# Chatit-cloud/BEE2BEE

Hardware: NVIDIA H100
Metric: decode_tokens_per_sec (higher is better)
Workload: dtype bf16

## Files before the change

bee2bee_b200/ops/__init__.py:

```python
from __future__ import annotations

import importlib
import importlib.util
from typing import Optional

import torch

EPI_PLAIN, EPI_RESIDUAL, EPI_GLU, EPI_QKV_ROPE, EPI_GELU = 0, 1, 2, 3, 4
PAGE = 64
NUM_SMS = 132

_C = None

LAUNCHES = [0]
_KERNEL_ENTRY_POINTS = ("add", "attention", "decode_advance", "embed", "fetch_window", "flag_signal", "flag_wait", "gemm",
                        "kv_append", "layernorm", "mark_seen", "quant_fp8_rows", "quant_mxfp8_rows", "rmsnorm", "sample",
                        "set_decode_state")


class _CountedModule:

    def __init__(self, mod):
        self._mod = mod
        for name in dir(mod):
# ... 287 lines not shown


def attention(q, k_cache, v_cache, out, block_table, q_start, q_len, kv_len, *, max_q, n_q, n_kv, head_dim,
              window=0, softcap=0.0, splits=1, ws=None, use_tc=-1, fq_out=None, fq_sf=None, fq_bn=0):
    native().attention(q, k_cache, v_cache, out, block_table, q_start, q_len, kv_len, ws, max_q, n_q, n_kv, head_dim,
                       window, softcap, splits, use_tc, _ptr(fq_out), _ptr(fq_sf), fq_bn)
    if splits > 1:
        LAUNCHES[0] += 1
    return out


def attention_fuses_quant(max_q: int, n_q: int, n_kv: int, head_dim: int, splits: int) -> bool:
    return native().attention_uses_tc(max_q, n_q, n_kv, head_dim) and (max_q > 1 or splits <= 1)


def set_attn_tc_min_q(n: int) -> None:
    native().set_attn_tc_min_q(int(n))


def get_attn_tc_min_q() -> int:
    return int(native().get_attn_tc_min_q())


def sample(logits, out_tokens, *, seen=None, temperature=None, top_p=None, rep_penalty=None, seeds=None, step=None,
           peer_tokens=0, history=0, hist_pos=None, hist_stride=0, signal_flag=0, signal_epoch=0, done_counter=0,
           vocab=0, softcap=0.0, row_map=0):
    native().sample(logits, seen, out_tokens, peer_tokens, history, hist_pos, hist_stride, vocab, softcap,
                    temperature, top_p,
                    rep_penalty, seeds, step, signal_flag, signal_epoch, done_counter, row_map)
    return out_tokens
# ... 5 lines not shown
```

csrc/attention_tc.cu:

```cuda
#include "kernels.h"

#include <cuda.h>
#include <cuda_fp8.h>

#include <cstdlib>
#include <type_traits>

#include "common.cuh"
#include "launch.cuh"
#include "wgmma.cuh"

namespace b2b {

int make_tmap_shared(CUtensorMap* m, const void* ptr, uint64_t rows, uint64_t cols, uint64_t ld, uint32_t box_rows,
                     int elt_bytes);

namespace {

constexpr int APAGE = 64;
constexpr int ATC_CONSUMERS = 256;
constexpr int ATC_THREADS = ATC_CONSUMERS + 32;
constexpr float LOG2E = 1.4426950408889634f;

struct AttnTcParams {
  __nv_bfloat16* out;
  const int* block_table;
  const int* q_start;
  const int* q_len;
  const int* kv_len;
  int max_pages, n_q, n_kv, window;
  float softcap;
  int splits, ws_rows;
  float* ws;
  uint8_t* q_out8;
  uint8_t* q_sf;
  int q_bn;
};

template <int D>
struct AtcCfg {
  static constexpr int BKV = 64;
  static constexpr int kQBytes = 128 * D * 2;
  static constexpr int kKVBytes = BKV * D * 2;
  static constexpr int kSmemBytes = kQBytes + 4 * kKVBytes + 256;
};

template <int D, bool SOFTCAP>
__global__ void __launch_bounds__(ATC_THREADS, 1)
attn_prefill_tc_kernel(const __grid_constant__ CUtensorMap tm_q, const __grid_constant__ CUtensorMap tm_k,
                       const __grid_constant__ CUtensorMap tm_v, const AttnTcParams p, const int G, const int QB) {
  using Cfg = AtcCfg<D>;
  constexpr int BKV = Cfg::BKV;
  constexpr int DB = D / 64;

  extern __shared__ __align__(1024) uint8_t smem[];
  if ((smem_u32(smem) & 1023u) != 0u) __trap();
  uint8_t* q_s = smem;
  uint8_t* k_s = q_s + Cfg::kQBytes;
  uint8_t* v_s = k_s + 2 * Cfg::kKVBytes;
  uint64_t* bars = reinterpret_cast<uint64_t*>(v_s + 2 * Cfg::kKVBytes);
  uint64_t* q_full = bars + 0;
  uint64_t* k_full = bars + 1;
  uint64_t* v_full = bars + 3;
  uint64_t* k_empty = bars + 5;
  uint64_t* v_empty = bars + 7;

  const int warp = threadIdx.x >> 5, lane = threadIdx.x & 31;
// ... 15 lines not shown
  const int qblk = split_mode ? 0 : gridDim.x - 1 - blockIdx.x;
  const int qlen = p.q_len[seq], kvlen = p.kv_len[seq];
  const int q0 = qblk * QB;
  bool active = q0 < qlen;
  const int nq_here = min(QB, qlen - q0);
  const int qtok0 = p.q_start[seq] + q0;
  const int pos0 = kvlen - qlen + q0;
  const int kv_hi = min(kvlen, pos0 + nq_here);
  const int kv_lo = p.window > 0 ? max(0, pos0 - p.window + 1) : 0;
  int t_lo = kv_lo / BKV, t_hi = (kv_hi + BKV - 1) / BKV;
  if (active && split_mode) {
    const int per = (t_hi - t_lo + p.splits - 1) / p.splits;
    t_lo = min(t_hi, t_lo + static_cast<int>(blockIdx.x) * per);
    t_hi = min(t_hi, t_lo + per);
    if (t_hi <= t_lo) {
      if (threadIdx.x < G) {
        float* w = p.ws + (((static_cast<size_t>(seq) * p.n_kv + kvh) * p.splits + blockIdx.x) * p.ws_rows + threadIdx.x) * (D + 2);
        for (int c = 0; c < D; ++c) w[c] = 0.f;
        w[D] = -INFINITY;
        w[D + 1] = 0.f;
      }
      active = false;
    }
  }
  const int nt = t_hi - t_lo;
  if (!active) return;

  if (warp == ATC_CONSUMERS / 32) {
    if (lane == 0) {
      mbar_arrive_expect_tx(q_full, Cfg::kQBytes);
      for (int g = 0; g < G; ++g)
        for (int c = 0; c < DB; ++c)
          tma_load_2d(q_s + c * (128 * 128) + g * QB * 128, &tm_q, q_full, (kvh * G + g) * D + c * 64, qtok0);
      const int* bt = p.block_table + static_cast<size_t>(seq) * p.max_pages;
      for (int n = 0; n < nt; ++n) {
        const int s = n & 1;
// ... 4 lines not shown
#pragma unroll
        for (int c = 0; c < DB; ++c)
          tma_load_2d(k_s + s * Cfg::kKVBytes + c * (BKV * 128), &tm_k, &k_full[s], kvh * D + c * 64, page * APAGE);
        mbar_wait(&v_empty[s], ph ^ 1u);
        mbar_arrive_expect_tx(&v_full[s], Cfg::kKVBytes);
#pragma unroll
        for (int c = 0; c < DB; ++c)
          tma_load_2d(v_s + s * Cfg::kKVBytes + c * (BKV * 128), &tm_v, &v_full[s], kvh * D + c * 64, page * APAGE);
      }
    }
    return;
  }

  const int wg = warp >> 2;
  const int ra = wg * 64 + (warp & 3) * 16 + (lane >> 2);
  int gq[2], iq[2], qpos[2];
  bool valid[2];
#pragma unroll
  for (int h = 0; h < 2; ++h) {
    const int row = ra + 8 * h;
    gq[h] = row / QB;
    iq[h] = row % QB;
    valid[h] = (gq[h] < G) && (iq[h] < nq_here);
    qpos[h] = pos0 + iq[h];
  }
  const float cap = p.softcap;
  const float inv_cap = SOFTCAP ? 1.f / cap : 0.f;
  float m_ref[2] = {-INFINITY, -INFINITY}, l[2] = {0.f, 0.f};
  float o[D / 2];
#pragma unroll
  for (int e = 0; e < D / 2; ++e) o[e] = 0.f;
  auto release = [&](uint64_t* bar) {
    __syncwarp();
    if (lane == 0) mbar_arrive(bar);
  };

  mbar_wait(q_full, 0);
  auto tile = [&](int n, auto masked) {
    const int t = t_lo + n, s = n & 1;
    const uint32_t ph = static_cast<uint32_t>((n >> 1) & 1);
    float sc[BKV / 2];
#pragma unroll
    for (int e = 0; e < BKV / 2; ++e) sc[e] = 0.f;
    mbar_wait(&k_full[s], ph);
    wgmma_fence();
#pragma unroll
    for (int kk = 0; kk < D / 16; ++kk) {
      const uint64_t a = make_sw128_kmajor_desc(smem_u32(q_s + (kk / 4) * (128 * 128) + wg * 64 * 128)) +
                         static_cast<uint64_t>((kk % 4) * 2);
      const uint64_t b = make_sw128_kmajor_desc(smem_u32(k_s + s * Cfg::kKVBytes + (kk / 4) * (BKV * 128))) +
                         static_cast<uint64_t>((kk % 4) * 2);
      Wgmma<BKV>::bf16_ss(sc, a, b, kk > 0 ? 1u : 0u);
    }
    wgmma_commit();
    wgmma_wait<0>();
    wgmma_fence_regs(sc);
    release(&k_empty[s]);

    float mrow[2] = {-INFINITY, -INFINITY};
#pragma unroll
    for (int e = 0; e < BKV / 2; ++e) {
      const int h = (e >> 1) & 1;
      float v = sc[e];
      if constexpr (SOFTCAP) v = cap * tanhf(v * inv_cap);
      v *= LOG2E;
      if constexpr (decltype(masked)::value) {
        const int kvpos = t * BKV + (e >> 2) * 8 + 2 * (lane & 3) + (e & 1);
        const bool ok = valid[h] && kvpos <= qpos[h] && kvpos < kvlen && (p.window <= 0 || kvpos > qpos[h] - p.window);
        v = ok ? v : -INFINITY;
      }
      sc[e] = v;
      mrow[h] = fmaxf(mrow[h], v);
    }
    float alpha[2], mr[2];
#pragma unroll
    for (int h = 0; h < 2; ++h) {
      mrow[h] = fmaxf(mrow[h], __shfl_xor_sync(0xffffffffu, mrow[h], 1));
      mrow[h] = fmaxf(mrow[h], __shfl_xor_sync(0xffffffffu, mrow[h], 2));
      alpha[h] = 1.f;
      if (mrow[h] > m_ref[h] + 8.f || (m_ref[h] == -INFINITY && mrow[h] > -INFINITY)) {
        alpha[h] = (m_ref[h] == -INFINITY) ? 0.f : exp2f(m_ref[h] - mrow[h]);
        m_ref[h] = mrow[h];
      }
      mr[h] = (m_ref[h] == -INFINITY) ? 0.f : m_ref[h];
    }
#pragma unroll
    for (int e = 0; e < D / 2; ++e) o[e] *= alpha[(e >> 1) & 1];
    uint32_t pa[BKV / 16][4];
    float lsum[2] = {0.f, 0.f};
#pragma unroll
    for (int e = 0; e < BKV / 2; e += 2) {
      const int h = (e >> 1) & 1;
      const float p0 = exp2f(sc[e] - mr[h]), p1 = exp2f(sc[e + 1] - mr[h]);
      lsum[h] += p0 + p1;
      const __nv_bfloat162 hv = __floats2bfloat162_rn(p0, p1);
      pa[e / 8][(e % 8) / 2] = *reinterpret_cast<const uint32_t*>(&hv);
    }
    l[0] = l[0] * alpha[0] + lsum[0];
    l[1] = l[1] * alpha[1] + lsum[1];
    mbar_wait(&v_full[s], ph);
    wgmma_fence_regs(o);
    wgmma_fence();
#pragma unroll
    for (int kk = 0; kk < BKV / 16; ++kk) {
      const uint64_t b = make_sw128_mnmajor_desc(smem_u32(v_s + s * Cfg::kKVBytes + kk * (16 * 128)), BKV * 128);
      Wgmma<D>::bf16_rs_tb(o, pa[kk], b, 1u);
    }
    wgmma_commit();
    wgmma_wait<0>();
    wgmma_fence_regs(o);
    release(&v_empty[s]);
  };

  for (int n = 0; n < nt; ++n) {
    const int t = t_lo + n;
    const bool full = nq_here == QB && (t + 1) * BKV - 1 <= pos0 && (t + 1) * BKV <= kvlen &&
                      (p.window <= 0 || t * BKV > pos0 + nq_here - 1 - p.window);
    if (full) tile(n, std::false_type{}); else tile(n, std::true_type{});
  }

#pragma unroll
  for (int h = 0; h < 2; ++h) {
    l[h] += __shfl_xor_sync(0xffffffffu, l[h], 1);
    l[h] += __shfl_xor_sync(0xffffffffu, l[h], 2);
  }
  const int c2 = 2 * (lane & 3);
#pragma unroll
  for (int h = 0; h < 2; ++h) {
    const float inv = l[h] > 0.f ? 1.f / l[h] : 0.f;
    const int tok = qtok0 + iq[h], head = kvh * G + gq[h];
    if (split_mode) {
      if (valid[h]) {
        float* wsrow = p.ws + (((static_cast<size_t>(seq) * p.n_kv + kvh) * p.splits + blockIdx.x) * p.ws_rows + gq[h]) * (D + 2);
        if ((lane & 3) == 0) {
          wsrow[D] = (m_ref[h] == -INFINITY) ? -INFINITY : m_ref[h] * 0.6931471805599453f;
          wsrow[D + 1] = l[h];
        }
#pragma unroll
        for (int j = 0; j < D / 8; ++j)
          *reinterpret_cast<float2*>(wsrow + 8 * j + c2) = make_float2(o[4 * j + 2 * h], o[4 * j + 2 * h + 1]);
      }
    } else if (p.q_out8 != nullptr) {
      const int ldq = p.n_q * D;
#pragma unroll
      for (int b = 0; b < D / 32; ++b) {
        float v[8];
        float amax = 0.f;
#pragma unroll
        for (int jj = 0; jj < 4; ++jj) {
          v[2 * jj] = bf16_round(o[4 * (4 * b + jj) + 2 * h] * inv);
          v[2 * jj + 1] = bf16_round(o[4 * (4 * b + jj) + 2 * h + 1] * inv);
          amax = fmaxf(amax, fmaxf(fabsf(v[2 * jj]), fabsf(v[2 * jj + 1])));
        }
        amax = fmaxf(amax, __shfl_xor_sync(0xffffffffu, amax, 1));
        amax = fmaxf(amax, __shfl_xor_sync(0xffffffffu, amax, 2));
        const uint32_t u = __float_as_uint(amax * (1.f / 448.f));
        int ex = static_cast<int>(u >> 23) - 127 + ((u & 0x7FFFFFu) ? 1 : 0);
        ex = max(-126, min(127, ex));
        const float scl = __uint_as_float(static_cast<uint32_t>(127 - ex) << 23);
        if (valid[h]) {
          const int feat = head * D + 32 * b;
          uint8_t* q8 = p.q_out8 + static_cast<size_t>(tok) * ldq + feat;
#pragma unroll
          for (int jj = 0; jj < 4; ++jj) {
            const uint16_t lo = __nv_cvt_float_to_fp8(v[2 * jj] * scl, __NV_SATFINITE, __NV_E4M3);
            const uint16_t hi = __nv_cvt_float_to_fp8(v[2 * jj + 1] * scl, __NV_SATFINITE, __NV_E4M3);
            *reinterpret_cast<uint16_t*>(q8 + 8 * jj + c2) = static_cast<uint16_t>(lo | (hi << 8));
          }
          if ((lane & 3) == 0) {
            const int tile_i = tok / p.q_bn, n = tok - tile_i * p.q_bn, rr = n & 127;
            p.q_sf[(static_cast<size_t>(tile_i) * (ldq >> 7) + (feat >> 7)) * (p.q_bn > 128 ? 1024 : 512) + (n >> 7) * 512 +
                   (rr & 31) * 16 + (rr >> 5) * 4 + ((feat >> 5) & 3)] = static_cast<uint8_t>(ex + 127);
          }
        }
      }
    } else if (valid[h]) {
      __nv_bfloat16* dst = p.out + (static_cast<size_t>(tok) * p.n_q + head) * D;
#pragma unroll
      for (int j = 0; j < D / 8; ++j)
        *reinterpret_cast<__nv_bfloat162*>(dst + 8 * j + c2) =
            __floats2bfloat162_rn(o[4 * j + 2 * h] * inv, o[4 * j + 2 * h + 1] * inv);
    }
  }
}

template <int D, bool SOFTCAP>
int launch_tc_cap(const CUtensorMap& tq, const CUtensorMap& tk, const CUtensorMap& tv, const AttnTcParams& p, int G, int QB,
                  int seqs, int qblocks, cudaStream_t s) {
  using Cfg = AtcCfg<D>;
  static bool set[64] = {};
  int dev = 0;
  cudaGetDevice(&dev);
  if (dev < 64 && !set[dev]) {
    cudaError_t e = cudaFuncSetAttribute(attn_prefill_tc_kernel<D, SOFTCAP>, cudaFuncAttributeMaxDynamicSharedMemorySize,
                                         Cfg::kSmemBytes);
    if (e != cudaSuccess) return static_cast<int>(e);
    set[dev] = true;
  }
  return static_cast<int>(launch_kernel(attn_prefill_tc_kernel<D, SOFTCAP>,
                                        dim3(p.splits > 1 ? p.splits : qblocks, p.n_kv, seqs), dim3(ATC_THREADS),
                                        Cfg::kSmemBytes, s, 1, tq, tk, tv, p, G, QB));
}

template <int D>
int launch_tc(const CUtensorMap& tq, const CUtensorMap& tk, const CUtensorMap& tv, const AttnTcParams& p, int G, int QB,
              int seqs, int qblocks, cudaStream_t s) {
  return p.softcap > 0.f ? launch_tc_cap<D, true>(tq, tk, tv, p, G, QB, seqs, qblocks, s)
                         : launch_tc_cap<D, false>(tq, tk, tv, p, G, QB, seqs, qblocks, s);
}

}

bool attention_tc_supported(int n_q, int n_kv, int head_dim) {
  if (n_kv <= 0 || n_q % n_kv) return false;
  const int G = n_q / n_kv;
  if (G != 1 && G != 2 && G != 4 && G != 8 && G != 16) return false;
  return head_dim == 64 || head_dim == 128 || head_dim == 256;
}

int launch_attention_tc(const void* q, const void* k_cache, const void* v_cache, void* out, const int* block_table,
                        const int* q_start, const int* q_len, const int* kv_len, int seqs, int max_q, int max_pages,
                        int n_tokens, int n_pages, int n_q, int n_kv, int head_dim, int window, float softcap,
                        int splits, float* ws, void* q_out8, void* q_sf, int q_bn, cudaStream_t s) {
  if (!attention_tc_supported(n_q, n_kv, head_dim)) return -2;
  const int G = n_q / n_kv, QB = 128 / G;
  CUtensorMap tq, tk, tv;
  int r = make_tmap_shared(&tq, q, static_cast<uint64_t>(n_tokens), static_cast<uint64_t>(n_q) * head_dim,
                           static_cast<uint64_t>(n_q) * head_dim, static_cast<uint32_t>(QB), 2);
  if (r) return r;
  const uint64_t kv_rows = static_cast<uint64_t>(n_pages) * APAGE, kv_cols = static_cast<uint64_t>(n_kv) * head_dim;
  if ((r = make_tmap_shared(&tk, k_cache, kv_rows, kv_cols, kv_cols, APAGE, 2))) return r;
  if ((r = make_tmap_shared(&tv, v_cache, kv_rows, kv_cols, kv_cols, APAGE, 2))) return r;
  AttnTcParams p;
  p.out = static_cast<__nv_bfloat16*>(out);
  p.block_table = block_table; p.q_start = q_start; p.q_len = q_len; p.kv_len = kv_len;
  p.max_pages = max_pages; p.n_q = n_q; p.n_kv = n_kv; p.window = window; p.softcap = softcap;
  p.splits = (max_q == 1 && splits > 1 && ws != nullptr) ? splits : 1;
  p.ws = ws;
  p.ws_rows = attn_rows(G, 1);
  p.q_out8 = p.splits > 1 ? nullptr : static_cast<uint8_t*>(q_out8);
  p.q_sf = static_cast<uint8_t*>(q_sf);
  p.q_bn = q_bn > 0 ? q_bn : 32;
  if (q_out8 != nullptr && p.splits > 1) return -8;
  const int qblocks = (max_q + QB - 1) / QB;
  int rc;
  switch (head_dim) {
    case 64: rc = launch_tc<64>(tq, tk, tv, p, G, QB, seqs, qblocks, s); break;
    case 128: rc = launch_tc<128>(tq, tk, tv, p, G, QB, seqs, qblocks, s); break;
    case 256: rc = launch_tc<256>(tq, tk, tv, p, G, QB, seqs, qblocks, s); break;
    default: return -3;
  }
  if (rc == 0 && p.splits > 1)
    rc = launch_attention_merge(out, q_start, q_len, ws, seqs, n_q, n_kv, head_dim, p.splits, s);
  return rc;
}

}
```

csrc/binding.cpp:

```cpp
#include <ATen/cuda/CUDAContext.h>
#include <c10/cuda/CUDAGuard.h>
#include <torch/extension.h>

#include "gemm_tc.cuh"
#include "kernels.h"
#include "launch.cuh"
#include "peer.h"

using at::Tensor;
using OptT = c10::optional<Tensor>;

namespace {

inline cudaStream_t cur_stream() { return at::cuda::getCurrentCUDAStream().stream(); }

inline void check(int err, const char* what) {
  if (err != 0) {
    const char* msg = err > 0 ? cudaGetErrorString(static_cast<cudaError_t>(err)) : "invalid argument";
    TORCH_CHECK(false, what, " failed: code ", err, " (", msg, ")");
  }
}
template <typename T>
inline T* ptr_or_null(const OptT& t) {
  return (t.has_value() && t->defined()) ? reinterpret_cast<T*>(t->data_ptr()) : nullptr;
// ... 270 lines not shown
          "attention_tc");
    return;
  }
  TORCH_CHECK(fq_out == 0, "fused output quantisation needs the tensor-core attention kernel");
  check(b2b::launch_attention(q.data_ptr(), k_cache.data_ptr(), v_cache.data_ptr(), out.data_ptr(),
                              reinterpret_cast<const int*>(block_table.data_ptr()),
                              reinterpret_cast<const int*>(q_start.data_ptr()),
                              reinterpret_cast<const int*>(q_len.data_ptr()),
                              reinterpret_cast<const int*>(kv_len.data_ptr()), ptr_or_null<float>(ws), seqs,
                              static_cast<int>(max_q), static_cast<int>(block_table.size(1)), static_cast<int>(n_q),
                              static_cast<int>(n_kv), static_cast<int>(head_dim), static_cast<int>(window),
                              static_cast<float>(softcap), static_cast<int>(splits), cur_stream()),
        "attention");
}

void sample(const Tensor& logits, const OptT& seen, const Tensor& out_tokens, int64_t peer_tokens,
            int64_t history, const OptT& hist_pos, int64_t hist_stride, int64_t vocab, double softcap,
            const OptT& temperature, const OptT& top_p,
            const OptT& rep_penalty, const OptT& seeds, const OptT& step, int64_t signal_flag, int64_t signal_epoch,
            int64_t done_counter, int64_t row_map) {
  TORCH_CHECK(logits.is_cuda() && logits.scalar_type() == at::kFloat && logits.stride(1) == 1, "logits: fp32");
  c10::cuda::CUDAGuard guard(logits.device());
  int* hp = ptr_or_null<int>(hist_pos);
  check(b2b::launch_sample(reinterpret_cast<const float*>(logits.data_ptr()), ptr_or_null<uint32_t>(seen),
                           reinterpret_cast<int*>(out_tokens.data_ptr()), as_ptr<int>(peer_tokens),
                           as_ptr<int>(history), hp, hp, static_cast<int>(hist_stride),
                           static_cast<int>(logits.size(0)), static_cast<int>(vocab > 0 ? vocab : logits.size(1)),
                           static_cast<int>(logits.stride(0)), static_cast<float>(softcap),
                           ptr_or_null<const float>(temperature), ptr_or_null<const float>(top_p),
                           ptr_or_null<const float>(rep_penalty), ptr_or_null<const uint32_t>(seeds),
// ... 95 lines not shown
  m.def("rmsnorm", &rmsnorm);
  m.def("layernorm", &layernorm);
  m.def("embed", &embed);
  m.def("kv_append", &kv_append);
  m.def("add", &add);
  m.def("quant_fp8_rows", &quant_fp8_rows);
  m.def("quant_mxfp8_rows", &quant_mxfp8_rows);
  m.def("flag_wait", &flag_wait);
  m.def("flag_signal", &flag_signal);
  m.def("decode_advance", &decode_advance);
  m.def("attention", &attention);
  m.def("attention_uses_tc", &attention_uses_tc, py::arg("max_q"), py::arg("n_q"), py::arg("n_kv"), py::arg("head_dim"),
        py::arg("use_tc") = -1);
  m.def("set_attn_tc_min_q", &set_attn_tc_min_q);
  m.def("get_attn_tc_min_q", &get_attn_tc_min_q);
  m.def("sample", &sample);
  m.def("sample_cluster_size", &sample_cluster_size, py::arg("batch"), py::arg("vocab"));
  m.def("mark_seen", &mark_seen);
  m.def("set_decode_state", &set_decode_state);
  m.def("fetch_window", &fetch_window);
  m.def("set_wait_policy", &set_wait_policy);
  m.def("peer_alloc", &peer_alloc);
  m.def("peer_free", &peer_free);
  m.def("ipc_export", &ipc_export);
  m.def("ipc_import", &ipc_import);
  m.def("ipc_close", &ipc_close);
  m.def("enable_peer_access", &enable_peer_access);
  m.def("can_access_peer", &can_access_peer);
  m.def("memcpy_peer", &memcpy_peer);
  m.def("host_ring_alloc", &host_ring_alloc);
// ... 4 lines not shown
```

csrc/gemm_tc.cu:

```cuda
#include "gemm_tc.cuh"

#include <cuda_fp8.h>

#include <cstdio>
#include <map>
#include <mutex>
#include <tuple>

#include "common.cuh"
#include "launch.cuh"
#include "wgmma.cuh"

namespace b2b {

constexpr int BM = 128;
constexpr int BK = 64;
constexpr int ROW_BYTES = 128;
constexpr int A_STAGE_BYTES = BM * ROW_BYTES;
constexpr int GEMM_CONSUMERS = 256;
constexpr int GEMM_THREADS = GEMM_CONSUMERS + 32;

template <int BN>
struct GemmCfg {
  static constexpr int kStages = (BN <= 32) ? 5 : (BN == 64 ? 4 : (BN == 128 ? 6 : 4));
// ... 630 lines not shown
  if ((r = set_attr_epi<BN, EPI_PLAIN>()) || (r = set_attr_epi<BN, EPI_RESIDUAL>()) || (r = set_attr_epi<BN, EPI_GLU>()) ||
      (r = set_attr_epi<BN, EPI_QKV_ROPE>()) || (r = set_attr_epi<BN, EPI_GELU>()))
    return r;
  return 0;
}
int gemm_tc_init() {
  int r = 0;
  if ((r = set_attr_bn<16>())) return r;
  if ((r = set_attr_bn<32>())) return r;
  if ((r = set_attr_bn<64>())) return r;
  if ((r = set_attr_bn<128>())) return r;
  if ((r = set_attr_bn<256>())) return r;
  return get_encode() ? 0 : -1;
}

int gemm_tc_default_stages(int bn) {
  switch (bn) {
    case 16: return GemmCfg<16>::kStages;
    case 32: return GemmCfg<32>::kStages;
    case 64: return GemmCfg<64>::kStages;
    case 128: return GemmCfg<128>::kStages;
    default: return GemmCfg<256>::kStages;
  }
}

int gemm_tc_max_splitk(int bn, int epi, int stages) {
  int ring;
  const int dflt = gemm_tc_default_stages(bn);
  if (stages <= 0 || stages > dflt) stages = dflt;
  if (stages < 2) stages = 2;
// ... 69 lines not shown
```

csrc/kernels.h:

```cpp
#pragma once
#include <cuda_runtime.h>
#include <stddef.h>
#include <stdint.h>

namespace b2b {

int launch_rmsnorm(const void* x, const void* gamma, const void* residual, void* out, float* rstd_out, int tokens,
                   int h, float eps, int gemma_plus_one, cudaStream_t s);
int launch_layernorm(const void* x, const void* gamma, const void* beta, void* out, int tokens, int h, float eps,
                     cudaStream_t s);
int launch_embed(const int* ids, const void* table, const void* pos_table, const int* positions, void* out, int tokens,
                 int h, int vocab, float scale, const uint32_t* tok_flag, const uint32_t* tok_epoch, const uint32_t* pf_flag,
                 const uint32_t* pf_need, cudaStream_t s);
int launch_kv_append(const void* qkv, void* q_out, void* k_cache, void* v_cache, const int* slots, int tokens,
                     int q_dim, int kv_dim, float q_scale, cudaStream_t s);
int launch_add(const void* a, const void* b, void* out, size_t n, cudaStream_t s);
int launch_quant_fp8_rows(const void* x, void* q, float* scale_out, int tokens, int h, float eps, int with_rms,
                          cudaStream_t s);
int launch_quant_mxfp8_rows(const void* x, void* q, void* sf, int tokens, int h, int bn, float eps, int with_rms,
                            float* sumsq_out, cudaStream_t s);
int launch_flag_wait(const uint32_t* flag, const uint32_t* epoch, uint32_t delta, cudaStream_t s);
int launch_decode_advance(int* positions, int* kv_len, int* slots, const int* q_len, const int* block_table,
                          int max_pages, int n, cudaStream_t s);
int launch_flag_signal(uint32_t* flag, uint32_t* epoch, uint32_t* bump_epoch, uint32_t* ack_flag, cudaStream_t s);

int launch_attention(const void* q, const void* k_cache, const void* v_cache, void* out, const int* block_table,
                     const int* q_start, const int* q_len, const int* kv_len, float* ws, int seqs, int max_q,
                     int max_pages, int n_q, int n_kv, int head_dim, int window, float softcap, int splits,
                     cudaStream_t s);
int attn_rows(int G, int QB);
bool attention_tc_supported(int n_q, int n_kv, int head_dim);
int launch_attention_tc(const void* q, const void* k_cache, const void* v_cache, void* out, const int* block_table,
                        const int* q_start, const int* q_len, const int* kv_len, int seqs, int max_q, int max_pages,
                        int n_tokens, int n_pages, int n_q, int n_kv, int head_dim, int window, float softcap,
                        int splits, float* ws, void* q_out8, void* q_sf, int q_bn, cudaStream_t s);
int launch_attention_merge(void* out, const int* q_start, const int* q_len, const float* ws, int seqs, int n_q, int n_kv,
                           int head_dim, int splits, cudaStream_t s);
int attention_init();

int launch_sample(const float* logits, uint32_t* seen, int* out_tokens, int* peer_tokens, int* history,
                  const int* hist_pos, int* hist_pos_out, int hist_stride, int batch, int vocab, int ld, float softcap,
                  const float* temperature, const float* top_p, const float* rep_penalty, const uint32_t* seeds,
                  const uint32_t* step, uint32_t* signal_flag, uint32_t* signal_epoch, uint32_t* done_counter,
                  const int* row_map, cudaStream_t s);
int sample_cluster_size(int batch, int vocab, int sms);
int launch_set_decode_state(int* positions, int* kv_len, int* q_len, const int* row_map, const int* kvlen, int n,
                            cudaStream_t s);
struct FlagWait { const uint32_t* flag; uint32_t target; uint32_t pad; };
int launch_fetch_window(const int* history, int hist_stride, const int* cursors, int rows, int width, int* out,
                        const FlagWait* waits, int n_waits, int* status, cudaStream_t s);
int launch_mark_seen(const int* ids, const int* seq_of, uint32_t* seen, int n, int vocab, cudaStream_t s);

int set_wait_policy_gemm(uint32_t* abort_word, unsigned long long limit_ns);
int set_wait_policy_elementwise(uint32_t* abort_word, unsigned long long limit_ns);

int gemm_tc_max_splitk(int bn, int epi, int stages);
int gemm_tc_init();

}
```

Baseline: 4840.

## Add dedicated single-warpgroup tensor-core decode attention kernel

New measurement: 4915, median of 6. 1.6% higher.

```diff
diff --git a/bee2bee_b200/ops/__init__.py b/bee2bee_b200/ops/__init__.py
--- a/bee2bee_b200/ops/__init__.py
+++ b/bee2bee_b200/ops/__init__.py
@@ -325,6 +325,14 @@
     return native().attention_uses_tc(max_q, n_q, n_kv, head_dim) and (max_q > 1 or splits <= 1)
 
 
+def decode_attention_attrs(head_dim: int, softcap: bool) -> dict:
+    return dict(native().decode_attention_attrs(int(head_dim), bool(softcap)))
+
+
+def gemm_bn32_attrs(epi: int) -> dict:
+    return dict(native().gemm_bn32_attrs(int(epi)))
+
+
 def set_attn_tc_min_q(n: int) -> None:
     native().set_attn_tc_min_q(int(n))
 
diff --git a/csrc/attention_tc.cu b/csrc/attention_tc.cu
--- a/csrc/attention_tc.cu
+++ b/csrc/attention_tc.cu
@@ -18,8 +18,11 @@
 namespace {
 
 constexpr int APAGE = 64;
+constexpr int BKV = 64;
 constexpr int ATC_CONSUMERS = 256;
 constexpr int ATC_THREADS = ATC_CONSUMERS + 32;
+constexpr int ADEC_CONSUMERS = 128;
+constexpr int ADEC_THREADS = ADEC_CONSUMERS + 32;
 constexpr float LOG2E = 1.4426950408889634f;
 
 struct AttnTcParams {
@@ -39,18 +42,197 @@
 
 template <int D>
 struct AtcCfg {
-  static constexpr int BKV = 64;
   static constexpr int kQBytes = 128 * D * 2;
   static constexpr int kKVBytes = BKV * D * 2;
   static constexpr int kSmemBytes = kQBytes + 4 * kKVBytes + 256;
 };
+
+template <int D>
+struct AdecCfg {
+  static constexpr int kQBytes = 64 * D * 2;
+  static constexpr int kKVBytes = BKV * D * 2;
+  static constexpr int kSmemBytes = kQBytes + 4 * kKVBytes + 256;
+};
+
+struct Rows {
+  int gq[2];
+  int tok[2];
+  int qpos[2];
+  bool valid[2];
+  float m_ref[2];
+  float l[2];
+};
+
+__device__ __forceinline__ void release_slot(uint64_t* bar, int lane) {
+  __syncwarp();
+  if (lane == 0) mbar_arrive(bar);
+}
+
+template <int D, bool SOFTCAP, bool MASKED>
+__device__ __forceinline__ void attn_tile(Rows& r, float (&o)[D / 2], const uint8_t* q_rows, int q_blk,
+                                          const uint8_t* k_tile, const uint8_t* v_tile, uint64_t* k_full,
+                                          uint64_t* v_full, uint64_t* k_empty, uint64_t* v_empty, uint32_t ph, int t,
+                                          int kvlen, int window, float cap, float inv_cap, int lane) {
+  float sc[BKV / 2];
+#pragma unroll
+  for (int e = 0; e < BKV / 2; ++e) sc[e] = 0.f;
+  mbar_wait(k_full, ph);
+  wgmma_fence();
+#pragma unroll
+  for (int kk = 0; kk < D / 16; ++kk) {
+    const uint64_t a = make_sw128_kmajor_desc(smem_u32(q_rows + (kk / 4) * q_blk)) + static_cast<uint64_t>((kk % 4) * 2);
+    const uint64_t b = make_sw128_kmajor_desc(smem_u32(k_tile + (kk / 4) * (BKV * 128))) +
+                       static_cast<uint64_t>((kk % 4) * 2);
+    Wgmma<BKV>::bf16_ss(sc, a, b, kk > 0 ? 1u : 0u);
+  }
+  wgmma_commit();
+  wgmma_wait<0>();
+  wgmma_fence_regs(sc);
+  release_slot(k_empty, lane);
+
+  float mrow[2] = {-INFINITY, -INFINITY};
+#pragma unroll
+  for (int e = 0; e < BKV / 2; ++e) {
+    const int h = (e >> 1) & 1;
+    float v = sc[e];
+    if constexpr (SOFTCAP) v = cap * tanhf(v * inv_cap);
+    v *= LOG2E;
+    if constexpr (MASKED) {
+      const int kvpos = t * BKV + (e >> 2) * 8 + 2 * (lane & 3) + (e & 1);
+      const bool ok = r.valid[h] && kvpos <= r.qpos[h] && kvpos < kvlen && (window <= 0 || kvpos > r.qpos[h] - window);
+      v = ok ? v : -INFINITY;
+    }
+    sc[e] = v;
+    mrow[h] = fmaxf(mrow[h], v);
+  }
+  float alpha[2], mr[2];
+#pragma unroll
+  for (int h = 0; h < 2; ++h) {
+    mrow[h] = fmaxf(mrow[h], __shfl_xor_sync(0xffffffffu, mrow[h], 1));
+    mrow[h] = fmaxf(mrow[h], __shfl_xor_sync(0xffffffffu, mrow[h], 2));
+    alpha[h] = 1.f;
+    if (mrow[h] > r.m_ref[h] + 8.f || (r.m_ref[h] == -INFINITY && mrow[h] > -INFINITY)) {
+      alpha[h] = (r.m_ref[h] == -INFINITY) ? 0.f : exp2f(r.m_ref[h] - mrow[h]);
+      r.m_ref[h] = mrow[h];
+    }
+    mr[h] = (r.m_ref[h] == -INFINITY) ? 0.f : r.m_ref[h];
+  }
+#pragma unroll
+  for (int e = 0; e < D / 2; ++e) o[e] *= alpha[(e >> 1) & 1];
+  uint32_t pa[BKV / 16][4];
+  float lsum[2] = {0.f, 0.f};
+#pragma unroll
+  for (int e = 0; e < BKV / 2; e += 2) {
+    const int h = (e >> 1) & 1;
+    const float p0 = exp2f(sc[e] - mr[h]), p1 = exp2f(sc[e + 1] - mr[h]);
+    lsum[h] += p0 + p1;
+    const __nv_bfloat162 hv = __floats2bfloat162_rn(p0, p1);
+    pa[e / 8][(e % 8) / 2] = *reinterpret_cast<const uint32_t*>(&hv);
+  }
+  r.l[0] = r.l[0] * alpha[0] + lsum[0];
+  r.l[1] = r.l[1] * alpha[1] + lsum[1];
+  mbar_wait(v_full, ph);
+  wgmma_fence_regs(o);
+  wgmma_fence();
+#pragma unroll
+  for (int kk = 0; kk < BKV / 16; ++kk) {
+    const uint64_t b = make_sw128_mnmajor_desc(smem_u32(v_tile + kk * (16 * 128)), BKV * 128);
+    Wgmma<D>::bf16_rs_tb(o, pa[kk], b, 1u);
+  }
+  wgmma_commit();
+  wgmma_wait<0>();
+  wgmma_fence_regs(o);
+  release_slot(v_empty, lane);
+}
+
+template <int D>
+__device__ __forceinline__ float* ws_row(const AttnTcParams& p, int seq, int kvh, int split, int g) {
+  return p.ws + (((static_cast<size_t>(seq) * p.n_kv + kvh) * p.splits + split) * p.ws_rows + g) * (D + 2);
+}
+
+template <int D>
+__device__ __forceinline__ void store_empty_partial(const AttnTcParams& p, int seq, int kvh, int split, int G) {
+  if (threadIdx.x < G) {
+    float* w = ws_row<D>(p, seq, kvh, split, threadIdx.x);
+    for (int c = 0; c < D; ++c) w[c] = 0.f;
+    w[D] = -INFINITY;
+    w[D + 1] = 0.f;
+  }
+}
+
+template <int D>
+__device__ __forceinline__ void store_rows(const AttnTcParams& p, Rows& r, const float (&o)[D / 2], int seq, int kvh,
+                                           int split, int G, int lane) {
+#pragma unroll
+  for (int h = 0; h < 2; ++h) {
+    r.l[h] += __shfl_xor_sync(0xffffffffu, r.l[h], 1);
+    r.l[h] += __shfl_xor_sync(0xffffffffu, r.l[h], 2);
+  }
+  const int c2 = 2 * (lane & 3);
+#pragma unroll
+  for (int h = 0; h < 2; ++h) {
+    const float inv = r.l[h] > 0.f ? 1.f / r.l[h] : 0.f;
+    const int tok = r.tok[h], head = kvh * G + r.gq[h];
+    if (p.splits > 1) {
+      if (r.valid[h]) {
+        float* wsrow = ws_row<D>(p, seq, kvh, split, r.gq[h]);
+        if ((lane & 3) == 0) {
+          wsrow[D] = (r.m_ref[h] == -INFINITY) ? -INFINITY : r.m_ref[h] * 0.6931471805599453f;
+          wsrow[D + 1] = r.l[h];
+        }
+#pragma unroll
+        for (int j = 0; j < D / 8; ++j)
+          *reinterpret_cast<float2*>(wsrow + 8 * j + c2) = make_float2(o[4 * j + 2 * h], o[4 * j + 2 * h + 1]);
+      }
+    } else if (p.q_out8 != nullptr) {
+      const int ldq = p.n_q * D;
+#pragma unroll
+      for (int b = 0; b < D / 32; ++b) {
+        float v[8];
+        float amax = 0.f;
+#pragma unroll
+        for (int jj = 0; jj < 4; ++jj) {
+          v[2 * jj] = bf16_round(o[4 * (4 * b + jj) + 2 * h] * inv);
+          v[2 * jj + 1] = bf16_round(o[4 * (4 * b + jj) + 2 * h + 1] * inv);
+          amax = fmaxf(amax, fmaxf(fabsf(v[2 * jj]), fabsf(v[2 * jj + 1])));
+        }
+        amax = fmaxf(amax, __shfl_xor_sync(0xffffffffu, amax, 1));
+        amax = fmaxf(amax, __shfl_xor_sync(0xffffffffu, amax, 2));
+        const uint32_t u = __float_as_uint(amax * (1.f / 448.f));
+        int ex = static_cast<int>(u >> 23) - 127 + ((u & 0x7FFFFFu) ? 1 : 0);
+        ex = max(-126, min(127, ex));
+        const float scl = __uint_as_float(static_cast<uint32_t>(127 - ex) << 23);
+        if (r.valid[h]) {
+          const int feat = head * D + 32 * b;
+          uint8_t* q8 = p.q_out8 + static_cast<size_t>(tok) * ldq + feat;
+#pragma unroll
+          for (int jj = 0; jj < 4; ++jj) {
+            const uint16_t lo = __nv_cvt_float_to_fp8(v[2 * jj] * scl, __NV_SATFINITE, __NV_E4M3);
+            const uint16_t hi = __nv_cvt_float_to_fp8(v[2 * jj + 1] * scl, __NV_SATFINITE, __NV_E4M3);
+            *reinterpret_cast<uint16_t*>(q8 + 8 * jj + c2) = static_cast<uint16_t>(lo | (hi << 8));
+          }
+          if ((lane & 3) == 0) {
+            const int tile_i = tok / p.q_bn, n = tok - tile_i * p.q_bn, rr = n & 127;
+            p.q_sf[(static_cast<size_t>(tile_i) * (ldq >> 7) + (feat >> 7)) * (p.q_bn > 128 ? 1024 : 512) + (n >> 7) * 512 +
+                   (rr & 31) * 16 + (rr >> 5) * 4 + ((feat >> 5) & 3)] = static_cast<uint8_t>(ex + 127);
+          }
+        }
+      }
+    } else if (r.valid[h]) {
+      __nv_bfloat16* dst = p.out + (static_cast<size_t>(tok) * p.n_q + head) * D;
+#pragma unroll
+      for (int j = 0; j < D / 8; ++j)
+        *reinterpret_cast<__nv_bfloat162*>(dst + 8 * j + c2) =
+            __floats2bfloat162_rn(o[4 * j + 2 * h] * inv, o[4 * j + 2 * h + 1] * inv);
+    }
+  }
+}
 
 template <int D, bool SOFTCAP>
 __global__ void __launch_bounds__(ATC_THREADS, 1)
 attn_prefill_tc_kernel(const __grid_constant__ CUtensorMap tm_q, const __grid_constant__ CUtensorMap tm_k,
                        const __grid_constant__ CUtensorMap tm_v, const AttnTcParams p, const int G, const int QB) {
   using Cfg = AtcCfg<D>;
-  constexpr int BKV = Cfg::BKV;
   constexpr int DB = D / 64;
 
   extern __shared__ __align__(1024) uint8_t smem[];
@@ -96,12 +278,7 @@
     t_lo = min(t_hi, t_lo + static_cast<int>(blockIdx.x) * per);
     t_hi = min(t_hi, t_lo + per);
     if (t_hi <= t_lo) {
-      if (threadIdx.x < G) {
-        float* w = p.ws + (((static_cast<size_t>(seq) * p.n_kv + kvh) * p.splits + blockIdx.x) * p.ws_rows + threadIdx.x) * (D + 2);
-        for (int c = 0; c < D; ++c) w[c] = 0.f;
-        w[D] = -INFINITY;
-        w[D + 1] = 0.f;
-      }
+      store_empty_partial<D>(p, seq, kvh, blockIdx.x, G);
       active = false;
     }
   }
@@ -136,174 +313,181 @@
 
   const int wg = warp >> 2;
   const int ra = wg * 64 + (warp & 3) * 16 + (lane >> 2);
-  int gq[2], iq[2], qpos[2];
-  bool valid[2];
+  Rows r;
 #pragma unroll
   for (int h = 0; h < 2; ++h) {
     const int row = ra + 8 * h;
-    gq[h] = row / QB;
-    iq[h] = row % QB;
-    valid[h] = (gq[h] < G) && (iq[h] < nq_here);
-    qpos[h] = pos0 + iq[h];
+    const int iq = row % QB;
+    r.gq[h] = row / QB;
+    r.tok[h] = qtok0 + iq;
+    r.valid[h] = (r.gq[h] < G) && (iq < nq_here);
+    r.qpos[h] = pos0 + iq;
+    r.m_ref[h] = -INFINITY;
+    r.l[h] = 0.f;
   }
   const float cap = p.softcap;
   const float inv_cap = SOFTCAP ? 1.f / cap : 0.f;
-  float m_ref[2] = {-INFINITY, -INFINITY}, l[2] = {0.f, 0.f};
   float o[D / 2];
 #pragma unroll
   for (int e = 0; e < D / 2; ++e) o[e] = 0.f;
-  auto release = [&](uint64_t* bar) {
-    __syncwarp();
-    if (lane == 0) mbar_arrive(bar);
-  };
 
   mbar_wait(q_full, 0);
-  auto tile = [&](int n, auto masked) {
+  const uint8_t* q_rows = q_s + wg * 64 * 128;
+  for (int n = 0; n < nt; ++n) {
     const int t = t_lo + n, s = n & 1;
     const uint32_t ph = static_cast<uint32_t>((n >> 1) & 1);
-    float sc[BKV / 2];
-#pragma unroll
-    for (int e = 0; e < BKV / 2; ++e) sc[e] = 0.f;
-    mbar_wait(&k_full[s], ph);
-    wgmma_fence();
-#pragma unroll
-    for (int kk = 0; kk < D / 16; ++kk) {
-      const uint64_t a = make_sw128_kmajor_desc(smem_u32(q_s + (kk / 4) * (128 * 128) + wg * 64 * 128)) +
-                         static_cast<uint64_t>((kk % 4) * 2);
-      const uint64_t b = make_sw128_kmajor_desc(smem_u32(k_s + s * Cfg::kKVBytes + (kk / 4) * (BKV * 128))) +
-                         static_cast<uint64_t>((kk % 4) * 2);
-      Wgmma<BKV>::bf16_ss(sc, a, b, kk > 0 ? 1u : 0u);
-    }
-    wgmma_commit();
-    wgmma_wait<0>();
-    wgmma_fence_regs(sc);
-    release(&k_empty[s]);
-
-    float mrow[2] = {-INFINITY, -INFINITY};
-#pragma unroll
-    for (int e = 0; e < BKV / 2; ++e) {
-      const int h = (e >> 1) & 1;
-      float v = sc[e];
-      if constexpr (SOFTCAP) v = cap * tanhf(v * inv_cap);
-      v *= LOG2E;
-      if constexpr (decltype(masked)::value) {
-        const int kvpos = t * BKV + (e >> 2) * 8 + 2 * (lane & 3) + (e & 1);
-        const bool ok = valid[h] && kvpos <= qpos[h] && kvpos < kvlen && (p.window <= 0 || kvpos > qpos[h] - p.window);
-        v = ok ? v : -INFINITY;
-      }
-      sc[e] = v;
-      mrow[h] = fmaxf(mrow[h], v);
-    }
-    float alpha[2], mr[2];
-#pragma unroll
-    for (int h = 0; h < 2; ++h) {
-      mrow[h] = fmaxf(mrow[h], __shfl_xor_sync(0xffffffffu, mrow[h], 1));
-      mrow[h] = fmaxf(mrow[h], __shfl_xor_sync(0xffffffffu, mrow[h], 2));
-      alpha[h] = 1.f;
-      if (mrow[h] > m_ref[h] + 8.f || (m_ref[h] == -INFINITY && mrow[h] > -INFINITY)) {
-        alpha[h] = (m_ref[h] == -INFINITY) ? 0.f : exp2f(m_ref[h] - mrow[h]);
-        m_ref[h] = mrow[h];
-      }
-      mr[h] = (m_ref[h] == -INFINITY) ? 0.f : m_ref[h];
-    }
-#pragma unroll
-    for (int e = 0; e < D / 2; ++e) o[e] *= alpha[(e >> 1) & 1];
-    uint32_t pa[BKV / 16][4];
-    float lsum[2] = {0.f, 0.f};
-#pragma unroll
-    for (int e = 0; e < BKV / 2; e += 2) {
-      const int h = (e >> 1) & 1;
-      const float p0 = exp2f(sc[e] - mr[h]), p1 = exp2f(sc[e + 1] - mr[h]);
-      lsum[h] += p0 + p1;
-      const __nv_bfloat162 hv = __floats2bfloat162_rn(p0, p1);
-      pa[e / 8][(e % 8) / 2] = *reinterpret_cast<const uint32_t*>(&hv);
-    }
-    l[0] = l[0] * alpha[0] + lsum[0];
-    l[1] = l[1] * alpha[1] + lsum[1];
-    mbar_wait(&v_full[s], ph);
-    wgmma_fence_regs(o);
-    wgmma_fence();
-#pragma unroll
-    for (int kk = 0; kk < BKV / 16; ++kk) {
-      const uint64_t b = make_sw128_mnmajor_desc(smem_u32(v_s + s * Cfg::kKVBytes + kk * (16 * 128)), BKV * 128);
-      Wgmma<D>::bf16_rs_tb(o, pa[kk], b, 1u);
-    }
-    wgmma_commit();
-    wgmma_wait<0>();
-    wgmma_fence_regs(o);
-    release(&v_empty[s]);
-  };
-
-  for (int n = 0; n < nt; ++n) {
-    const int t = t_lo + n;
     const bool full = nq_here == QB && (t + 1) * BKV - 1 <= pos0 && (t + 1) * BKV <= kvlen &&
                       (p.window <= 0 || t * BKV > pos0 + nq_here - 1 - p.window);
-    if (full) tile(n, std::false_type{}); else tile(n, std::true_type{});
-  }
-
+    const uint8_t* kt = k_s + s * Cfg::kKVBytes;
+    const uint8_t* vt = v_s + s * Cfg::kKVBytes;
+    if (full)
+      attn_tile<D, SOFTCAP, false>(r, o, q_rows, 128 * 128, kt, vt, &k_full[s], &v_full[s], &k_empty[s], &v_empty[s], ph,
+                                   t, kvlen, p.window, cap, inv_cap, lane);
+    else
+      attn_tile<D, SOFTCAP, true>(r, o, q_rows, 128 * 128, kt, vt, &k_full[s], &v_full[s], &k_empty[s], &v_empty[s], ph,
+                                  t, kvlen, p.window, cap, inv_cap, lane);
+  }
+  store_rows<D>(p, r, o, seq, kvh, blockIdx.x, G, lane);
+}
+
+struct DecItem {
+  int seq, kvh, split, qtok, qpos, kvlen, t_lo, t_hi;
+  bool empty_share;
+};
+
+__device__ __forceinline__ bool decode_item(const AttnTcParams& p, int item, DecItem& it) {
+  it.split = item % p.splits;
+  const int rest = item / p.splits;
+  it.kvh = rest % p.n_kv;
+  it.seq = rest / p.n_kv;
+  const int qlen = p.q_len[it.seq];
+  it.kvlen = p.kv_len[it.seq];
+  it.empty_share = false;
+  if (qlen <= 0) return false;
+  it.qtok = p.q_start[it.seq];
+  it.qpos = it.kvlen - qlen;
+  const int kv_hi = min(it.kvlen, it.qpos + 1);
+  const int kv_lo = p.window > 0 ? max(0, it.qpos - p.window + 1) : 0;
+  it.t_lo = kv_lo / BKV;
+  it.t_hi = (kv_hi + BKV - 1) / BKV;
+  if (p.splits > 1) {
+    const int per = (it.t_hi - it.t_lo + p.splits - 1) / p.splits;
+    it.t_lo = min(it.t_hi, it.t_lo + it.split * per);
+    it.t_hi = min(it.t_hi, it.t_lo + per);
+    if (it.t_hi <= it.t_lo) {
+      it.empty_share = true;
+      return false;
+    }
+  }
+  return true;
+}
+
+template <int D, bool SOFTCAP>
+__global__ void __launch_bounds__(ADEC_THREADS, 1)
+attn_decode_tc_kernel(const __grid_constant__ CUtensorMap tm_q, const __grid_constant__ CUtensorMap tm_k,
+                      const __grid_constant__ CUtensorMap tm_v, const AttnTcParams p, const int G) {
+  using Cfg = AdecCfg<D>;
+  constexpr int DB = D / 64;
+
+  extern __shared__ __align__(1024) uint8_t smem[];
+  if ((smem_u32(smem) & 1023u) != 0u) __trap();
+  uint8_t* q_s = smem;
+  uint8_t* k_s = q_s + Cfg::kQBytes;
+  uint8_t* v_s = k_s + 2 * Cfg::kKVBytes;
+  uint64_t* bars = reinterpret_cast<uint64_t*>(v_s + 2 * Cfg::kKVBytes);
+  uint64_t* q_full = bars + 0;
+  uint64_t* k_full = bars + 1;
+  uint64_t* v_full = bars + 3;
+  uint64_t* k_empty = bars + 5;
+  uint64_t* v_empty = bars + 7;
+
+  const int warp = threadIdx.x >> 5, lane = threadIdx.x & 31;
+  if (threadIdx.x == ADEC_CONSUMERS) {
+    mbar_init(q_full, 1);
+    for (int i = 0; i < 2; ++i) {
+      mbar_init(&k_full[i], 1); mbar_init(&v_full[i], 1);
+      mbar_init(&k_empty[i], ADEC_CONSUMERS / 32); mbar_init(&v_empty[i], ADEC_CONSUMERS / 32);
+    }
+    fence_barrier_init();
+    tma_prefetch_desc(&tm_q); tma_prefetch_desc(&tm_k); tma_prefetch_desc(&tm_v);
+  }
+  __syncthreads();
+
+  pdl_wait();
+  DecItem it;
+  if (!decode_item(p, blockIdx.x, it)) {
+    if (it.empty_share) store_empty_partial<D>(p, it.seq, it.kvh, it.split, G);
+    return;
+  }
+
+  if (warp == ADEC_CONSUMERS / 32) {
+    if (lane == 0) {
+      mbar_arrive_expect_tx(q_full, Cfg::kQBytes);
+      for (int c = 0; c < DB; ++c)
+        tma_load_2d(q_s + c * (64 * 128), &tm_q, q_full, c * 64, it.qtok * p.n_q + it.kvh * G);
+      const int* bt = p.block_table + static_cast<size_t>(it.seq) * p.max_pages;
+      for (int n = 0; n < it.t_hi - it.t_lo; ++n) {
+        const int s = n & 1;
+        const uint32_t ph = static_cast<uint32_t>((n >> 1) & 1);
+        const int page = bt[it.t_lo + n];
+        mbar_wait(&k_empty[s], ph ^ 1u);
+        mbar_arrive_expect_tx(&k_full[s], Cfg::kKVBytes);
+#pragma unroll
+        for (int c = 0; c < DB; ++c)
+          tma_load_2d(k_s + s * Cfg::kKVBytes + c * (BKV * 128), &tm_k, &k_full[s], it.kvh * D + c * 64, page * APAGE);
+        mbar_wait(&v_empty[s], ph ^ 1u);
+        mbar_arrive_expect_tx(&v_full[s], Cfg::kKVBytes);
+#pragma unroll
+        for (int c = 0; c < DB; ++c)
+          tma_load_2d(v_s + s * Cfg::kKVBytes + c * (BKV * 128), &tm_v, &v_full[s], it.kvh * D + c * 64, page * APAGE);
+      }
+    }
+    return;
+  }
+
+  const int ra = warp * 16 + (lane >> 2);
+  Rows r;
 #pragma unroll
   for (int h = 0; h < 2; ++h) {
-    l[h] += __shfl_xor_sync(0xffffffffu, l[h], 1);
-    l[h] += __shfl_xor_sync(0xffffffffu, l[h], 2);
-  }
-  const int c2 = 2 * (lane & 3);
-#pragma unroll
-  for (int h = 0; h < 2; ++h) {
-    const float inv = l[h] > 0.f ? 1.f / l[h] : 0.f;
-    const int tok = qtok0 + iq[h], head = kvh * G + gq[h];
-    if (split_mode) {
-      if (valid[h]) {
-        float* wsrow = p.ws + (((static_cast<size_t>(seq) * p.n_kv + kvh) * p.splits + blockIdx.x) * p.ws_rows + gq[h]) * (D + 2);
-        if ((lane & 3) == 0) {
-          wsrow[D] = (m_ref[h] == -INFINITY) ? -INFINITY : m_ref[h] * 0.6931471805599453f;
-          wsrow[D + 1] = l[h];
-        }
-#pragma unroll
-        for (int j = 0; j < D / 8; ++j)
-          *reinterpret_cast<float2*>(wsrow + 8 * j + c2) = make_float2(o[4 * j + 2 * h], o[4 * j + 2 * h + 1]);
-      }
-    } else if (p.q_out8 != nullptr) {
-      const int ldq = p.n_q * D;
-#pragma unroll
-      for (int b = 0; b < D / 32; ++b) {
-        float v[8];
-        float amax = 0.f;
-#pragma unroll
-        for (int jj = 0; jj < 4; ++jj) {
-          v[2 * jj] = bf16_round(o[4 * (4 * b + jj) + 2 * h] * inv);
-          v[2 * jj + 1] = bf16_round(o[4 * (4 * b + jj) + 2 * h + 1] * inv);
-          amax = fmaxf(amax, fmaxf(fabsf(v[2 * jj]), fabsf(v[2 * jj + 1])));
-        }
-        amax = fmaxf(amax, __shfl_xor_sync(0xffffffffu, amax, 1));
-        amax = fmaxf(amax, __shfl_xor_sync(0xffffffffu, amax, 2));
-        const uint32_t u = __float_as_uint(amax * (1.f / 448.f));
-        int ex = static_cast<int>(u >> 23) - 127 + ((u & 0x7FFFFFu) ? 1 : 0);
-        ex = max(-126, min(127, ex));
-        const float scl = __uint_as_float(static_cast<uint32_t>(127 - ex) << 23);
-        if (valid[h]) {
-          const int feat = head * D + 32 * b;
-          uint8_t* q8 = p.q_out8 + static_cast<size_t>(tok) * ldq + feat;
-#pragma unroll
-          for (int jj = 0; jj < 4; ++jj) {
-            const uint16_t lo = __nv_cvt_float_to_fp8(v[2 * jj] * scl, __NV_SATFINITE, __NV_E4M3);
-            const uint16_t hi = __nv_cvt_float_to_fp8(v[2 * jj + 1] * scl, __NV_SATFINITE, __NV_E4M3);
-            *reinterpret_cast<uint16_t*>(q8 + 8 * jj + c2) = static_cast<uint16_t>(lo | (hi << 8));
-          }
-          if ((lane & 3) == 0) {
-            const int tile_i = tok / p.q_bn, n = tok - tile_i * p.q_bn, rr = n & 127;
-            p.q_sf[(static_cast<size_t>(tile_i) * (ldq >> 7) + (feat >> 7)) * (p.q_bn > 128 ? 1024 : 512) + (n >> 7) * 512 +
-                   (rr & 31) * 16 + (rr >> 5) * 4 + ((feat >> 5) & 3)] = static_cast<uint8_t>(ex + 127);
-          }
-        }
-      }
-    } else if (valid[h]) {
-      __nv_bfloat16* dst = p.out + (static_cast<size_t>(tok) * p.n_q + head) * D;
-#pragma unroll
-      for (int j = 0; j < D / 8; ++j)
-        *reinterpret_cast<__nv_bfloat162*>(dst + 8 * j + c2) =
-            __floats2bfloat162_rn(o[4 * j + 2 * h] * inv, o[4 * j + 2 * h + 1] * inv);
-    }
-  }
+    r.gq[h] = ra + 8 * h;
+    r.tok[h] = it.qtok;
+    r.valid[h] = r.gq[h] < G;
+    r.qpos[h] = it.qpos;
+    r.m_ref[h] = -INFINITY;
+    r.l[h] = 0.f;
+  }
+  const float cap = p.softcap;
+  const float inv_cap = SOFTCAP ? 1.f / cap : 0.f;
+  float o[D / 2];
+#pragma unroll
+  for (int e = 0; e < D / 2; ++e) o[e] = 0.f;
+  mbar_wait(q_full, 0);
+  for (int n = 0; n < it.t_hi - it.t_lo; ++n) {
+    const int t = it.t_lo + n, s = n & 1;
+    const uint32_t ph = static_cast<uint32_t>((n >> 1) & 1);
+    const bool full = (t + 1) * BKV - 1 <= it.qpos && (t + 1) * BKV <= it.kvlen &&
+                      (p.window <= 0 || t * BKV > it.qpos - p.window);
+    const uint8_t* kt = k_s + s * Cfg::kKVBytes;
+    const uint8_t* vt = v_s + s * Cfg::kKVBytes;
+    if (full)
+      attn_tile<D, SOFTCAP, false>(r, o, q_s, 64 * 128, kt, vt, &k_full[s], &v_full[s], &k_empty[s], &v_empty[s], ph, t,
+                                   it.kvlen, p.window, cap, inv_cap, lane);
+    else
+      attn_tile<D, SOFTCAP, true>(r, o, q_s, 64 * 128, kt, vt, &k_full[s], &v_full[s], &k_empty[s], &v_empty[s], ph, t,
+                                  it.kvlen, p.window, cap, inv_cap, lane);
+  }
+  pdl_launch_dependents();
+  store_rows<D>(p, r, o, it.seq, it.kvh, it.split, G, lane);
+}
+
+template <typename K>
+cudaError_t set_smem_once(K kernel, int bytes, bool (&set)[64]) {
+  int dev = 0;
+  cudaGetDevice(&dev);
+  if (dev < 64 && set[dev]) return cudaSuccess;
+  const cudaError_t e = cudaFuncSetAttribute(kernel, cudaFuncAttributeMaxDynamicSharedMemorySize, bytes);
+  if (e == cudaSuccess && dev < 64) set[dev] = true;
+  return e;
 }
 
 template <int D, bool SOFTCAP>
@@ -311,17 +495,24 @@
                   int seqs, int qblocks, cudaStream_t s) {
   using Cfg = AtcCfg<D>;
   static bool set[64] = {};
-  int dev = 0;
-  cudaGetDevice(&dev);
-  if (dev < 64 && !set[dev]) {
-    cudaError_t e = cudaFuncSetAttribute(attn_prefill_tc_kernel<D, SOFTCAP>, cudaFuncAttributeMaxDynamicSharedMemorySize,
-                                         Cfg::kSmemBytes);
-    if (e != cudaSuccess) return static_cast<int>(e);
-    set[dev] = true;
-  }
+  const cudaError_t e = set_smem_once(attn_prefill_tc_kernel<D, SOFTCAP>, Cfg::kSmemBytes, set);
+  if (e != cudaSuccess) return static_cast<int>(e);
   return static_cast<int>(launch_kernel(attn_prefill_tc_kernel<D, SOFTCAP>,
                                         dim3(p.splits > 1 ? p.splits : qblocks, p.n_kv, seqs), dim3(ATC_THREADS),
                                         Cfg::kSmemBytes, s, 1, tq, tk, tv, p, G, QB));
+}
+
+template <int D, bool SOFTCAP>
+int launch_decode_cap(const CUtensorMap& tq, const CUtensorMap& tk, const CUtensorMap& tv, const AttnTcParams& p, int G,
+                      int seqs, cudaStream_t s) {
+  using Cfg = AdecCfg<D>;
+  static bool set[64] = {};
+  const cudaError_t e = set_smem_once(attn_decode_tc_kernel<D, SOFTCAP>, Cfg::kSmemBytes, set);
+  if (e != cudaSuccess) return static_cast<int>(e);
+  const int items = seqs * p.n_kv * p.splits;
+  if (items <= 0) return 0;
+  return static_cast<int>(launch_kernel(attn_decode_tc_kernel<D, SOFTCAP>, dim3(items), dim3(ADEC_THREADS),
+                                        Cfg::kSmemBytes, s, 1, tq, tk, tv, p, G));
 }
 
 template <int D>
@@ -331,6 +522,26 @@
                          : launch_tc_cap<D, false>(tq, tk, tv, p, G, QB, seqs, qblocks, s);
 }
 
+template <int D>
+int launch_decode(const CUtensorMap& tq, const CUtensorMap& tk, const CUtensorMap& tv, const AttnTcParams& p, int G,
+                  int seqs, cudaStream_t s) {
+  return p.softcap > 0.f ? launch_decode_cap<D, true>(tq, tk, tv, p, G, seqs, s)
+                         : launch_decode_cap<D, false>(tq, tk, tv, p, G, seqs, s);
+}
+
+template <int D, bool SOFTCAP>
+int decode_attrs_cap(KernelAttrs* a) {
+  cudaFuncAttributes fa;
+  const cudaError_t e = cudaFuncGetAttributes(&fa, attn_decode_tc_kernel<D, SOFTCAP>);
+  if (e != cudaSuccess) return static_cast<int>(e);
+  a->regs = fa.numRegs;
+  a->static_smem = static_cast<int>(fa.sharedSizeBytes);
+  a->dynamic_smem = AdecCfg<D>::kSmemBytes;
+  a->local_bytes = static_cast<int>(fa.localSizeBytes);
+  a->threads = ADEC_THREADS;
+  return 0;
+}
+
 }
 
 bool attention_tc_supported(int n_q, int n_kv, int head_dim) {
@@ -338,6 +549,14 @@
   const int G = n_q / n_kv;
   if (G != 1 && G != 2 && G != 4 && G != 8 && G != 16) return false;
   return head_dim == 64 || head_dim == 128 || head_dim == 256;
+}
+
+int attention_tc_decode_attrs(int head_dim, int softcap, KernelAttrs* a) {
+  switch (head_dim) {
+    case 64: return softcap ? decode_attrs_cap<64, true>(a) : decode_attrs_cap<64, false>(a);
+    case 128: return softcap ? decode_attrs_cap<128, true>(a) : decode_attrs_cap<128, false>(a);
+    default: return -3;
+  }
 }
 
 int launch_attention_tc(const void* q, const void* k_cache, const void* v_cache, void* out, const int* block_table,
@@ -346,9 +565,12 @@
                         int splits, float* ws, void* q_out8, void* q_sf, int q_bn, cudaStream_t s) {
   if (!attention_tc_supported(n_q, n_kv, head_dim)) return -2;
   const int G = n_q / n_kv, QB = 128 / G;
+  const bool decode = max_q == 1 && head_dim <= 128;
   CUtensorMap tq, tk, tv;
-  int r = make_tmap_shared(&tq, q, static_cast<uint64_t>(n_tokens), static_cast<uint64_t>(n_q) * head_dim,
-                           static_cast<uint64_t>(n_q) * head_dim, static_cast<uint32_t>(QB), 2);
+  int r = decode ? make_tmap_shared(&tq, q, static_cast<uint64_t>(n_tokens) * n_q, static_cast<uint64_t>(head_dim),
+                                    static_cast<uint64_t>(head_dim), 64, 2)
+                 : make_tmap_shared(&tq, q, static_cast<uint64_t>(n_tokens), static_cast<uint64_t>(n_q) * head_dim,
+                                    static_cast<uint64_t>(n_q) * head_dim, static_cast<uint32_t>(QB), 2);
   if (r) return r;
   const uint64_t kv_rows = static_cast<uint64_t>(n_pages) * APAGE, kv_cols = static_cast<uint64_t>(n_kv) * head_dim;
   if ((r = make_tmap_shared(&tk, k_cache, kv_rows, kv_cols, kv_cols, APAGE, 2))) return r;
@@ -367,8 +589,8 @@
   const int qblocks = (max_q + QB - 1) / QB;
   int rc;
   switch (head_dim) {
-    case 64: rc = launch_tc<64>(tq, tk, tv, p, G, QB, seqs, qblocks, s); break;
-    case 128: rc = launch_tc<128>(tq, tk, tv, p, G, QB, seqs, qblocks, s); break;
+    case 64: rc = decode ? launch_decode<64>(tq, tk, tv, p, G, seqs, s) : launch_tc<64>(tq, tk, tv, p, G, QB, seqs, qblocks, s); break;
+    case 128: rc = decode ? launch_decode<128>(tq, tk, tv, p, G, seqs, s) : launch_tc<128>(tq, tk, tv, p, G, QB, seqs, qblocks, s); break;
     case 256: rc = launch_tc<256>(tq, tk, tv, p, G, QB, seqs, qblocks, s); break;
     default: return -3;
   }
diff --git a/csrc/binding.cpp b/csrc/binding.cpp
--- a/csrc/binding.cpp
+++ b/csrc/binding.cpp
@@ -308,6 +308,27 @@
         "attention");
 }
 
+py::dict attrs_dict(const b2b::KernelAttrs& a) {
+  py::dict d;
+  d["regs"] = a.regs;
+  d["static_smem"] = a.static_smem;
+  d["dynamic_smem"] = a.dynamic_smem;
+  d["local_bytes"] = a.local_bytes;
+  d["threads"] = a.threads;
+  return d;
+}
+
+py::dict decode_attention_attrs(int64_t head_dim, bool softcap) {
+  b2b::KernelAttrs a{};
+  check(b2b::attention_tc_decode_attrs(static_cast<int>(head_dim), softcap ? 1 : 0, &a), "decode_attention_attrs");
+  return attrs_dict(a);
+}
+py::dict gemm_bn32_attrs(int64_t epi) {
+  b2b::KernelAttrs a{};
+  check(b2b::gemm_tc_bn32_attrs(static_cast<int>(epi), &a), "gemm_bn32_attrs");
+  return attrs_dict(a);
+}
+
 void sample(const Tensor& logits, const OptT& seen, const Tensor& out_tokens, int64_t peer_tokens,
             int64_t history, const OptT& hist_pos, int64_t hist_stride, int64_t vocab, double softcap,
             const OptT& temperature, const OptT& top_p,
@@ -433,6 +454,8 @@
         py::arg("use_tc") = -1);
   m.def("set_attn_tc_min_q", &set_attn_tc_min_q);
   m.def("get_attn_tc_min_q", &get_attn_tc_min_q);
+  m.def("decode_attention_attrs", &decode_attention_attrs, py::arg("head_dim"), py::arg("softcap"));
+  m.def("gemm_bn32_attrs", &gemm_bn32_attrs, py::arg("epi"));
   m.def("sample", &sample);
   m.def("sample_cluster_size", &sample_cluster_size, py::arg("batch"), py::arg("vocab"));
   m.def("mark_seen", &mark_seen);
diff --git a/csrc/gemm_tc.cu b/csrc/gemm_tc.cu
--- a/csrc/gemm_tc.cu
+++ b/csrc/gemm_tc.cu
@@ -8,6 +8,7 @@
 #include <tuple>
 
 #include "common.cuh"
+#include "kernels.h"
 #include "launch.cuh"
 #include "wgmma.cuh"
 
@@ -668,6 +669,29 @@
   return get_encode() ? 0 : -1;
 }
 
+template <int EPI>
+static int bn32_attrs(KernelAttrs* a) {
+  cudaFuncAttributes fa;
+  const cudaError_t e = cudaFuncGetAttributes(&fa, gemm_tc_kernel<32, EPI, 0>);
+  if (e != cudaSuccess) return static_cast<int>(e);
+  a->regs = fa.numRegs;
+  a->static_smem = static_cast<int>(fa.sharedSizeBytes);
+  a->dynamic_smem = GemmCfg<32>::kSmemBytes;
+  a->local_bytes = static_cast<int>(fa.localSizeBytes);
+  a->threads = GEMM_THREADS;
+  return 0;
+}
+int gemm_tc_bn32_attrs(int epi, KernelAttrs* a) {
+  switch (epi) {
+    case EPI_PLAIN: return bn32_attrs<EPI_PLAIN>(a);
+    case EPI_RESIDUAL: return bn32_attrs<EPI_RESIDUAL>(a);
+    case EPI_GLU: return bn32_attrs<EPI_GLU>(a);
+    case EPI_QKV_ROPE: return bn32_attrs<EPI_QKV_ROPE>(a);
+    case EPI_GELU: return bn32_attrs<EPI_GELU>(a);
+    default: return -4;
+  }
+}
+
 int gemm_tc_default_stages(int bn) {
   switch (bn) {
     case 16: return GemmCfg<16>::kStages;
diff --git a/csrc/kernels.h b/csrc/kernels.h
--- a/csrc/kernels.h
+++ b/csrc/kernels.h
@@ -29,7 +29,11 @@
                      int max_pages, int n_q, int n_kv, int head_dim, int window, float softcap, int splits,
                      cudaStream_t s);
 int attn_rows(int G, int QB);
+
+struct KernelAttrs { int regs, static_smem, dynamic_smem, local_bytes, threads; };
+
 bool attention_tc_supported(int n_q, int n_kv, int head_dim);
+int attention_tc_decode_attrs(int head_dim, int softcap, KernelAttrs* a);
 int launch_attention_tc(const void* q, const void* k_cache, const void* v_cache, void* out, const int* block_table,
                         const int* q_start, const int* q_len, const int* kv_len, int seqs, int max_q, int max_pages,
                         int n_tokens, int n_pages, int n_q, int n_kv, int head_dim, int window, float softcap,
@@ -56,5 +60,6 @@
 
 int gemm_tc_max_splitk(int bn, int epi, int stages);
 int gemm_tc_init();
+int gemm_tc_bn32_attrs(int epi, KernelAttrs* a);
 
 }
```
